# leodd/Lifted-Hybrid-Variational-Inference

Hardware: AMD Instinct MI355X
Metric: lbp_sweeps_per_sec_10M_edge_hybrid_mrf (higher is better)
Workload: dtype f64

## Files before the change

### include/lhvi.h

```cpp
#ifndef LHVI_H
#define LHVI_H

#include <stddef.h>
#include <stdint.h>

#ifdef __cplusplus
extern "C" {
#endif

#define LHVI_ABI_VERSION 31
#define LHVI_MAX_ARITY 6

#define LHVI_OK 0
#define LHVI_E_ARG (-1)
#define LHVI_E_LAUNCH (-2)
#define LHVI_E_UNSUPPORTED (-3)
#define LHVI_E_NODEVICE (-4)
#define LHVI_E_NOT_PD (-5)

#define LHVI_POT_GENERIC 0
#define LHVI_POT_TABLE 1
#define LHVI_POT_GAUSSIAN 2
#define LHVI_POT_QUADRATIC 3
#define LHVI_POT_HYBRID_QUADRATIC 4
#define LHVI_POT_LINEAR_GAUSSIAN 5
#define LHVI_POT_X2 6
#define LHVI_POT_XY 7
#define LHVI_POT_MLN 8
#define LHVI_POT_MLN_HARD 9
#define LHVI_POT_IMAGE_NODE 10
#define LHVI_POT_IMAGE_EDGE 11

typedef struct lhvi_graph {
    int32_t V, F, E, nnz;
    const int32_t* fac_ptr;
    const int32_t* edge_var;
    const int32_t* edge_fac;
    const int32_t* edge_canon;
    const int32_t* var_ptr;
    const int32_t* var_edge;
    const double* edge_count;
    const int32_t* fac_pot;
    const double* var_value;
    const int32_t* var_dom;
    const double* var_mult;
    const double* fac_mult;
    int32_t D;
    const int32_t* dom_cont;
    const double* dom_lo;
    const double* dom_hi;
    const int32_t* dom_ptr;
    const double* dom_val;
    const double* edge_value;
    const int32_t* slot_var;
    const int32_t* hub_vars;
    int32_t n_hubs;
} lhvi_graph_t;
#define LHVI_HUB_DEGREE 64

typedef struct lhvi_pots {
    int32_t P;
    const int32_t* kind;
    const int32_t* off;
    const double* param;
    int32_t interpreted;
} lhvi_pots_t;

int lhvi_version(void);
const char* lhvi_strerror(int code);
int lhvi_last_hip_error(void);
int lhvi_device_count(void);


int lhvi_gabp_init(const lhvi_graph_t* g, double* f2v, double* v2f, void* stream);
int lhvi_gabp_v2f(const lhvi_graph_t* g, const double* f2v, double* v2f, void* stream);
int lhvi_gabp_f2v(const lhvi_graph_t* g, const lhvi_pots_t* pots, const double* v2f, double* f2v, void* stream);
int lhvi_gabp_run(const lhvi_graph_t* g, const lhvi_pots_t* pots, double* f2v, double* v2f, int iterations, void* stream);
typedef struct lhvi_gabp_plan {
    const int32_t* pslot;
    const int32_t* info;
    const double* count;
    int32_t n_hub_rows;
    const int32_t* rec;
    const double* pot_words;
    const int32_t* seg;
    int32_t n_seg;
} lhvi_gabp_plan_t;
size_t lhvi_gabp_pull_workspace_bytes(const lhvi_graph_t* g);
int lhvi_gabp_pull(const lhvi_graph_t* g, const lhvi_pots_t* pots, const lhvi_gabp_plan_t* plan, const double* v_prev,
                   double* v_next, int first, void* stream);
int lhvi_gabp_run_pull(const lhvi_graph_t* g, const lhvi_pots_t* pots, const lhvi_gabp_plan_t* plan, double* f2v, double* v2f,
                       int iterations, void* ws, size_t ws_bytes, void* stream);

int lhvi_gabp_graph_create(const lhvi_graph_t* g, const lhvi_pots_t* pots, const lhvi_gabp_plan_t* plan, double* f2v, double* v2f,
                           double* mu_var, int iterations, void* ws, size_t ws_bytes, void** handle_out);
int lhvi_gabp_graph_launch(void* handle, void* stream);
int lhvi_gabp_graph_destroy(void* handle);

int lhvi_gabp_marginals(const lhvi_graph_t* g, const double* f2v, double* mu_var, void* stream);

size_t lhvi_log_likelihood_workspace_bytes(const lhvi_graph_t* g);
int lhvi_log_likelihood(const lhvi_graph_t* g, const lhvi_pots_t* pots, const double* x, double* out, void* ws, size_t ws_bytes,
                        void* stream);


#define LHVI_PBP_EP 1u
#define LHVI_PBP_EPBP_DISCRETE 2u
#define LHVI_PBP_SKIP_TERMS 16u
#define LHVI_PBP_LEAVE_ROOM 256u
#define LHVI_PBP_CQ 512u
#define LHVI_PBP_BOUNDARY_TOTALS 2048u
#define LHVI_PBP_NO_UNIQ 4096u
#define LHVI_PBP_V2F_RECORDS 8192u
#define LHVI_PBP_WIDE_PAIRS 16384u
#define LHVI_PBP_SHARE_CUS 32768u
#define LHVI_PBP_NO_GRID 128u
#define LHVI_PBP_FUSED_RECORDS16 131072u
#define LHVI_PBP_F2V_HEAVY 262144u
#define LHVI_PBP_F2V_SMALL 524288u
#define LHVI_PBP_F2V_PAIR 1048576u
#define LHVI_PBP_F2V_FAST 2097152u
#define LHVI_PBP_F2V_CQ 4194304u
#define LHVI_PBP_F2V_GENERIC 8388608u
#define LHVI_PBP_F2V_ALL (LHVI_PBP_F2V_HEAVY | LHVI_PBP_F2V_SMALL | LHVI_PBP_F2V_PAIR | LHVI_PBP_F2V_FAST | LHVI_PBP_F2V_CQ | LHVI_PBP_F2V_GENERIC)
#define LHVI_PBP_POW2_GROUPS 65536u

typedef struct lhvi_pbp {
    int32_t n;
    int32_t T;
    uint32_t flags;
    double var_threshold;
    double max_log_value;
    const double* particles;
    const double* old_particles;
    const int32_t* np;
    const uint8_t* uniq;
    const double* q;
    const int32_t* fast_edges;
    int32_t n_fast;
    const int32_t* generic_edges;
    int32_t n_generic;
    int32_t generic_pts_log2;
    const void* fast_desc;
    const void* heavy_desc;
    int32_t n_heavy;
    const void* light_desc;
    int32_t n_light;
    const int32_t* bslot;
    const int32_t* brow_ptr;
    const int64_t* brow_off;
    const int32_t* brow_peer;
    const double* recv;
    int32_t rank;
    const double* var_degree;
    int32_t var_lo, var_hi;
    uint32_t* f2v_ticket;
    const int32_t* prop_desc;
    int32_t n_prop_desc;
    const void* pair_desc;
    int32_t n_pair;
    const void* cq_desc;
    int32_t n_cq;
    const int32_t* v2f_wide;
    int32_t n_v2f_wide;
    const int32_t* v2f_narrow;
    int32_t n_v2f_narrow;
    const int32_t* v2f_hub;
    int32_t n_v2f_hub;
    const int32_t* v2f_mid16;
    int32_t n_v2f_mid16;
    const int32_t* v2f_mid32;
    int32_t n_v2f_mid32;
    const int32_t* prop_hub;
    int32_t n_prop_hub;
    double* prop_partial;
    const int32_t* resample_vars;
    int32_t n_resample_vars;
    const void* small16_desc;
    int32_t n_small16;
    const void* small32_desc;
    int32_t n_small32;
    const int64_t* halo_off;
    double* halo_buf;
} lhvi_pbp_t;

#define LHVI_PBP_DESC_BYTES 128
#define LHVI_PBP_TICKET_WORDS 16
#define LHVI_PBP_TICKET_COUNTERS 8
int lhvi_pbp_describe(const lhvi_graph_t* g, const lhvi_pots_t* pots, const lhvi_pbp_t* s, const int32_t* edges, int32_t count,
                      void* desc_out, void* stream);
int lhvi_pbp_describe_cq(const lhvi_graph_t* g, const lhvi_pots_t* pots, const lhvi_pbp_t* s, const int32_t* edges, int32_t count,
                         void* desc_out, void* stream);
int lhvi_pbp_var_sum(const lhvi_graph_t* g, const lhvi_pbp_t* s, const double* f2v, double* out, void* stream);
int lhvi_pbp_domain_grid(const lhvi_graph_t* g, const lhvi_pbp_t* s, double* x, void* stream);
int lhvi_pbp_refine_grid(const lhvi_graph_t* g, const lhvi_pbp_t* s, const double* logb, double* x, double* best, double* best_val,
                         void* stream);
int lhvi_debug_exp(const double* x, double* y, int64_t n, void* stream);
int lhvi_debug_exp_acc(const double* x, const double* c, double* y, int64_t n, void* stream);
int lhvi_debug_exp_acc_floor(const double* x, const double* c, double* y, int64_t n, void* stream);
// ... 409 lines not shown
```

### lifted-hybrid-variational-inference_amd/csrc/fastmath.hpp

```cpp
#pragma once
#include "common.hpp"

namespace lhvi {

#include "exp_table.inc"
constexpr int EXP_TAB_N = 1 << LHVI_EXP_TABLE_BITS;

__device__ __forceinline__ double exp_core(double t, const double* __restrict__ tab ) {
    const double MAGIC = LHVI_SCONST(6755399441055744.0);
    const double u = fma(t, LHVI_SCONST(LHVI_EXP_INV_STEP), MAGIC);
    const int nn = __double2loint(u);
    const double kd = u - MAGIC;
    double r = fma(kd, LHVI_SCONST(-LHVI_EXP_STEP_HI), t);
    r = fma(kd, LHVI_SCONST(-LHVI_EXP_STEP_LO), r);
    double p = fma(r, LHVI_SCONST(1.6666666666666666667e-1), 0.5);
    p = fma(p, r, 1.0);
    p = fma(p, r, 1.0);
    return ldexp(tab[nn & (EXP_TAB_N - 1)] * p, nn >> LHVI_EXP_TABLE_BITS);
}

__device__ __forceinline__ void load_exp_table(double* __restrict__ tab) {
    for (int i = threadIdx.x; i < EXP_TAB_N; i += blockDim.x) tab[i] = EXP_TAB[i];
    __syncthreads();
}

struct ExpShift { double magic, scale; };

__device__ __forceinline__ ExpShift exp_shift(double C) {
    const double MAGIC = 6755399441055744.0;
    ExpShift o;
    o.magic = fma(C, LHVI_EXP_INV_STEP, MAGIC);
    const double kd = o.magic - MAGIC;
    double r = fma(kd, -LHVI_EXP_STEP_HI, C);
    r = fma(kd, -LHVI_EXP_STEP_LO, r);
    double p = fma(r, 1.6666666666666666667e-1, 0.5);
    p = fma(p, r, 1.0);
    o.scale = fma(p, r, 1.0);
    return o;
}

__device__ __forceinline__ double exp_accumulate(double acc, double t, double magic, const double* __restrict__ tab) {
    double u;
    asm("v_fma_f64 %0, %1, %2, %3" : "=v"(u) : "v"(t), "s"((double)LHVI_EXP_INV_STEP), "v"(magic));
    const int nn = __double2loint(u);
    const double kd = u - magic;
    const double r = fma(kd, -LHVI_EXP_STEP_HI, t);
    double p = fma(r, 1.6666666666666666667e-1, 0.5);
    p = fma(p, r, 1.0);
    p = fma(p, r, 1.0);
    return fma(ldexp(tab[nn & (EXP_TAB_N - 1)], nn >> LHVI_EXP_TABLE_BITS), p, acc);
}

struct ExpShiftFloor { double magic, scale; };

__device__ __forceinline__ void round_down_on() { asm volatile("s_setreg_imm32_b32 hwreg(HW_REG_MODE, 2, 2), 2\n\ts_nop 1" ::: "memory"); }
__device__ __forceinline__ void round_down_off() { asm volatile("s_setreg_imm32_b32 hwreg(HW_REG_MODE, 2, 2), 0\n\ts_nop 1" ::: "memory"); }

__device__ __forceinline__ ExpShiftFloor exp_shift_floor(double C) {
    const double MAGIC = 6755399441055744.0;
    ExpShiftFloor o;
    const double m = fma(C, LHVI_EXP_INV_STEP, MAGIC);
    const double kd = m - MAGIC;
    double r = fma(kd, -LHVI_EXP_STEP_HI, C);
    r = fma(kd, -LHVI_EXP_STEP_LO, r);
    double p = fma(r, 1.6666666666666666667e-1, 0.5);
    p = fma(p, r, 1.0);
    o.scale = fma(p, r, 1.0) * LHVI_EXPF_SCALE;
    o.magic = 844424930131968.0 + (kd - (double)(24 << LHVI_EXP_TABLE_BITS));
    return o;
}

__device__ __forceinline__ double exp_accumulate_floor(double acc, double s, double magic, const double* __restrict__ tab) {
    double u;
    asm volatile("v_add_f64 %0, %1, %2" : "=v"(u) : "v"(s), "v"(magic));
    const int nn = __double2loint(u);
    const double f = __builtin_amdgcn_fract(s);
    double p = fma(f, LHVI_SCONST(LHVI_EXPF_RHO), 1.0);
    p = fma(p, f, LHVI_SCONST(LHVI_EXPF_K1));
    p = fma(p, f, LHVI_SCONST(LHVI_EXPF_K0));
    const double entry = *reinterpret_cast<const double*>(reinterpret_cast<const char*>(tab) + (nn & ((EXP_TAB_N - 1) << 3)));
    return fma(ldexp(entry, nn >> (LHVI_EXP_TABLE_BITS + 3)), p, acc);
}

constexpr int LOG_TAB_N = 1 << LHVI_LOG_TABLE_BITS;
struct LogRec { double inv_c, log_c; };

__device__ __forceinline__ void load_log_table(LogRec* __restrict__ tab) {
    for (int i = threadIdx.x; i < LOG_TAB_N; i += blockDim.x) { tab[i].inv_c = LOG_TAB[2 * i]; tab[i].log_c = LOG_TAB[2 * i + 1]; }
}

__device__ __forceinline__ double log_table(double x, const LogRec* __restrict__ tab) {
    const int e = __builtin_amdgcn_frexp_exp(x);
    const double m = __builtin_amdgcn_frexp_mant(x);
    const LogRec c = tab[(__double2hiint(m) >> (20 - LHVI_LOG_TABLE_BITS)) & (LOG_TAB_N - 1)];
    const double r = fma(m, c.inv_c, -1.0);
    double q = fma(r, LHVI_SCONST(1.0 / 7.0), LHVI_SCONST(-1.0 / 6.0));
    q = fma(q, r, LHVI_SCONST(1.0 / 5.0));
    q = fma(q, r, -0.25);
    q = fma(q, r, LHVI_SCONST(1.0 / 3.0));
    q = fma(q, r, -0.5);
    const double l = fma(r * r, q, r);
    const double y = fma((double)e, LHVI_SCONST(LHVI_LN2), c.log_c + l);
    return x == __builtin_huge_val() ? x : y;
}

}
```

### lifted-hybrid-variational-inference_amd/csrc/pbp.hip

```cpp
#include "common.hpp"
#include "potential.hpp"
#include "fastmath.hpp"
#include "cq.hpp"
#include "gk21.hpp"

namespace lhvi {

__device__ __forceinline__ double wave_sum(double v) { return dpp_wave_reduce(v, SumOp()); }
__device__ __forceinline__ double wave_max(double v) { return dpp_wave_reduce(v, MaxOp()); }
__device__ __forceinline__ int wave_sum_i(int v) {
#pragma unroll
    for (int off = 32; off > 0; off >>= 1) v += __shfl_xor(v, off);
    return v;
}

constexpr double PAD_LOG_TERM = -6.0e5;

__host__ __device__ __forceinline__ int var_first(const lhvi_pbp_t& s) { return s.var_hi > s.var_lo ? s.var_lo : 0; }
__host__ __device__ __forceinline__ int var_limit(const lhvi_graph_t& g, const lhvi_pbp_t& s) { return s.var_hi > s.var_lo ? s.var_hi : g.V; }

__device__ __forceinline__ double norm_pdf_std(double x, double mu, double sig) {
    const double u = (x - mu) / sig;
    return exp(-u * u * 0.5) / (2.506628274631 * sig);
}
// ... 507 lines not shown
            d.pad[0] = cont_target ? 1 : 2;
        }
    }
    return d;
}

__global__ void __launch_bounds__(BLOCK) pbp_describe_kernel(lhvi_graph_t g, lhvi_pots_t pots, lhvi_pbp_t s,
                                                            const int32_t* __restrict__ edges, int count,
                                                            FastDesc* __restrict__ out) {
    const int i = blockIdx.x * BLOCK + threadIdx.x;
    if (i < count) out[i] = make_fast_desc(g, pots, s, edges[i]);
}

#define LHVI_WAVE_SYNC() do { __builtin_amdgcn_fence(__ATOMIC_ACQ_REL, "wavefront"); __builtin_amdgcn_wave_barrier(); } while (0)

enum { MODE_CONST = 0, MODE_VARK = 1, MODE_DISC = 2 };
struct AB { double a, b; };

template <int MODE>
__device__ __forceinline__ double fast_term(double acc, const AB* __restrict__ sh, const double* __restrict__ shk,
                                            const double* __restrict__ tab, int j, double X1, double X2, double magic) {
    const AB r = sh[j];
    double t;
    if (MODE == MODE_VARK) t = fma(shk[j], X2, fma(r.b, X1, r.a));
    else t = fma(r.b, fma(r.b, X2, X1), r.a);
    return exp_accumulate(acc, t, magic, tab);
}

template <int MODE>
__device__ __forceinline__ double fast_accumulate_uniform(const AB* __restrict__ sh, const double* __restrict__ shk,
                                                          const double* __restrict__ tab, int jn_, double X1, double X2, double C) {
    const int jn = __builtin_amdgcn_readfirstlane(jn_);
    const ExpShift sft = exp_shift(C);
    double acc0 = 0.0, acc1 = 0.0;
    int j = 0;
    for (; j + 2 <= jn; j += 2) {
        acc0 = fast_term<MODE>(acc0, sh, shk, tab, j, X1, X2, sft.magic);
        acc1 = fast_term<MODE>(acc1, sh, shk, tab, j + 1, X1, X2, sft.magic);
    }
    if (j < jn) acc0 = fast_term<MODE>(acc0, sh, shk, tab, j, X1, X2, sft.magic);
    return (acc0 + acc1) * sft.scale;
}

#define LHVI_PIN1(a) do { if (PIN) asm volatile("" : "+v"(a)); } while (0)
#define LHVI_PIN2(a, b) do { if (PIN) asm volatile("" : "+v"(a), "+v"(b)); } while (0)
template <int UNROLL = 4, bool PIN = false>
__device__ __forceinline__ double fast_accumulate_floor(const AB* __restrict__ sh, const double* __restrict__ tab, int jn_, double X1,
                                                        double C) {
    const int jn = __builtin_amdgcn_readfirstlane(jn_);
    LHVI_PIN1(C);
    ExpShiftFloor sft = exp_shift_floor(C);
    LHVI_PIN2(sft.magic, sft.scale);
    double acc0 = 0.0, acc1 = 0.0;
    int j = 0;
    round_down_on();
    if (UNROLL == 4) {
        double acc2 = 0.0, acc3 = 0.0;
        for (; j + 4 <= jn; j += 4) {
            const AB r0 = sh[j], r1 = sh[j + 1], r2 = sh[j + 2], r3 = sh[j + 3];
            acc0 = exp_accumulate_floor(acc0, fma(r0.b, X1, r0.a), sft.magic, tab);
            acc1 = exp_accumulate_floor(acc1, fma(r1.b, X1, r1.a), sft.magic, tab);
            acc2 = exp_accumulate_floor(acc2, fma(r2.b, X1, r2.a), sft.magic, tab);
            acc3 = exp_accumulate_floor(acc3, fma(r3.b, X1, r3.a), sft.magic, tab);
        }
        if (j < jn) { const AB r0 = sh[j]; acc0 = exp_accumulate_floor(acc0, fma(r0.b, X1, r0.a), sft.magic, tab); }
        if (j + 1 < jn) { const AB r1 = sh[j + 1]; acc1 = exp_accumulate_floor(acc1, fma(r1.b, X1, r1.a), sft.magic, tab); }
        if (j + 2 < jn) { const AB r2 = sh[j + 2]; acc2 = exp_accumulate_floor(acc2, fma(r2.b, X1, r2.a), sft.magic, tab); }
        acc0 += acc2; acc1 += acc3;
        LHVI_PIN2(acc0, acc1);
        round_down_off();
        return (acc0 + acc1) * sft.scale;
    }
    for (; j + 2 <= jn; j += 2) {
        const AB r0 = sh[j], r1 = sh[j + 1];
        acc0 = exp_accumulate_floor(acc0, fma(r0.b, X1, r0.a), sft.magic, tab);
        acc1 = exp_accumulate_floor(acc1, fma(r1.b, X1, r1.a), sft.magic, tab);
    }
    if (j < jn) { const AB r0 = sh[j]; acc0 = exp_accumulate_floor(acc0, fma(r0.b, X1, r0.a), sft.magic, tab); }
    LHVI_PIN2(acc0, acc1);
    round_down_off();
    return (acc0 + acc1) * sft.scale;
}

__global__ void __launch_bounds__(BLOCK) pbp_f2v_fast_kernel(lhvi_graph_t g, lhvi_pots_t pots, lhvi_pbp_t s,
                                                            const double* __restrict__ v2f, double* __restrict__ f2v,
                                                            const FastDesc* __restrict__ descs,
                                                            const double* __restrict__ param) {
    __shared__ AB sh_all[BLOCK / WAVE][WAVE];
    __shared__ double shk_all[BLOCK / WAVE][WAVE];
    __shared__ double sh_tab[EXP_TAB_N];
    __shared__ LogRec sh_log[LOG_TAB_N];
    load_log_table(sh_log);
    load_exp_table(sh_tab);
    const int wid = __builtin_amdgcn_readfirstlane(threadIdx.x >> 6);
    const int lane = threadIdx.x & 63;
    AB* sh = sh_all[wid];
    double* shk = shk_all[wid];
    const int nitems = s.fast_edges ? s.n_fast : g.E;
    const int nwaves = gridDim.x * (BLOCK / WAVE);
    const int n = s.n, S = s.n + s.T;
    for (int item = blockIdx.x * (BLOCK / WAVE) + wid; item < nitems; item += nwaves) {
        FastDesc d;
        if (descs) d = descs[item];
        else d = make_fast_desc(g, pots, s, s.fast_edges ? s.fast_edges[item] : item);
        if (d.cls != EDGE_FAST_CONT && d.cls != EDGE_FAST_DISC) continue;
        const double* __restrict__ par = param + d.par_off;
        const int np = d.np, npts = d.np + d.T, nj = d.nj;
        const bool partner_hidden = is_hidden(d.pval);
        double* out = f2v + (int64_t)d.e * S;

        double y0 = d.pval, m0 = 0.0;
        if (partner_hidden && lane < nj) { y0 = s.old_particles[(int64_t)d.pv * n + lane]; m0 = v2f[(int64_t)d.pce * n + lane]; }
        double xr[2] = {0.0, 0.0};
#pragma unroll
        for (int r = 0; r < 2; ++r) {
            const int rem = npts - 64 * r;
            if (rem > 0) {
                int lw = 6;
                if (rem <= 32) { lw = 0; while ((1 << lw) < rem) ++lw; }
                const int pl = lane & ((1 << lw) - 1), pp = 64 * r + pl;
                if (pl < rem) xr[r] = pp < np ? s.particles[(int64_t)d.tv * n + pp] : g.dom_val[d.gb + pp - np];
            }
        }

        const int mode = d.cls == EDGE_FAST_DISC ? MODE_DISC : (d.kind == LHVI_POT_HYBRID_QUADRATIC ? MODE_VARK : MODE_CONST);
        double kconst = 0.0;
        if (mode == MODE_CONST) { Quad2 q; quad2_of(d.kind, par, 0, q); kconst = d.pos == 0 ? q.a00 : q.a11; }
        auto stage = [&](int j0, int jn, double y, double m) {
            LHVI_WAVE_SYNC();
            {
                AB r;
                r.a = PAD_LOG_TERM; r.b = 0.0;
                double kk = 0.0;
                if (lane < jn) {
                    if (d.cls == EDGE_FAST_CONT) {
                        Quad2 q;
                        quad2_of(d.kind, par, (d.kind == LHVI_POT_HYBRID_QUADRATIC) ? (int)y : 0, q);
                        if (d.pos == 0) { r.a = (q.a11 * y + q.b1) * y + q.c + m; r.b = q.axy * y + q.b0; kk = q.a00; }
                        else            { r.a = (q.a00 * y + q.b0) * y + q.c + m; r.b = q.axy * y + q.b1; kk = q.a11; }
                    } else { r.a = m; r.b = y; }
                }
                if (mode == MODE_CONST) { r.a *= LHVI_EXP_INV_STEP; r.b *= LHVI_EXP_INV_STEP; }
                sh[lane] = r;
                if (mode == MODE_VARK) shk[lane] = kk;
            }
            LHVI_WAVE_SYNC();
        };
        const bool single_tile = nj <= 64;
        if (single_tile) stage(0, nj, y0, m0);

        for (int p0 = 0; p0 < npts; p0 += 64) {
            const int rem = npts - p0;
            int lw = 6;
            if (rem <= 32) { lw = 0; while ((1 << lw) < rem) ++lw; }
            const int width = 1 << lw, split = 64 >> lw, sub = lane >> lw, pl = lane & (width - 1);
            const int p = p0 + pl;
            const bool valid = pl < rem;
            double xv = 0.0;
            if (p0 == 0) xv = xr[0];
            else if (p0 == 64) xv = xr[1];
            else if (valid) xv = p < np ? s.particles[(int64_t)d.tv * n + p] : g.dom_val[d.gb + p - np];
            double X1 = 0.0, X2 = 0.0, C = 0.0;
            if (valid) {
                if (d.cls == EDGE_FAST_CONT) { X1 = xv; X2 = xv * xv; C = kconst * X2; }
                else {
                    const int nst = (int)par[2];
// ... 332 lines not shown
                                                             double* __restrict__ f2v, const HeavyDesc* __restrict__ descs,
                                                             int nitems) {
    __shared__ AB sh_all[HEAVY_BLOCK / WAVE][WAVE];
    __shared__ double sh_tab[EXP_TAB_N];
    __shared__ LogRec sh_log[LOG_TAB_N];
    load_log_table(sh_log);
    load_exp_table(sh_tab);
    const int wid = __builtin_amdgcn_readfirstlane(threadIdx.x >> 6);
    const int lane = threadIdx.x & 63;
    AB* sh = sh_all[wid];
    const int n = s.n, S = s.n + s.T;
    WorkCursor<8, HEAVY_BLOCK / WAVE> cur;
    const auto ticket = [] { return heavy_arg_reload<uint32_t*>(offsetof(HeavyArgs, f2v_ticket)); };
    if (!cur.start(ticket, nitems, lane)) return;
    int n_grid = 0, n_direct = 0;
    struct { int32_t e, nj, np, T, gb, grid; double ay, by, c, axy, bx, kx, gx0, gh; } d;
    HeavyHead hn = descs[cur.item].h;
    HeavyData h = heavy_fetch(hn, s, v2f, lane);
    for (;;) {
        d.e = hn.e; d.nj = hn.nj; d.np = hn.np; d.T = hn.T; d.gb = hn.gb; d.grid = hn.grid;
        {
            const HeavyCoef k = descs[cur.item].k;
            d.ay = k.ay; d.by = k.by; d.c = k.c; d.axy = k.axy; d.bx = k.bx; d.kx = k.kx; d.gx0 = k.gx0; d.gh = k.gh;
        }
        const int nxt = cur.next();
        const bool more = nxt < cur.limit;
        hn = descs[__builtin_amdgcn_readfirstlane(min(nxt, cur.limit - 1))].h;
        const int np = d.np, nj = d.nj;
        const auto out = scalar_row(f2v + (int64_t)d.e * S);
        const double kconst = d.kx;
        const bool eligible = grid_eligible(d.grid, nj, d.T);
        bool grid_path = eligible && !(s.flags & (LHVI_PBP_SKIP_TERMS | LHVI_PBP_NO_GRID));
        AB mine;
        mine.a = PAD_LOG_TERM; mine.b = 0.0;
        LHVI_WAVE_SYNC();
        {
            if (lane < nj) {
                const double y = h.y;
                mine.a = (d.ay * y + d.by) * y + d.c + h.m;
                mine.b = d.axy * y + d.bx;
            }
            AB scaled;
            scaled.a = mine.a * LHVI_EXP_INV_STEP; scaled.b = mine.b * LHVI_EXP_INV_STEP;
            sh[lane] = scaled;
        }
        LHVI_WAVE_SYNC();
        if (grid_path) {
            const double X = fmax(fabs(d.gx0), fabs(fma((double)(d.T - 1), d.gh, d.gx0)));
            const double bound = fma(fabs(mine.b) + fabs(kconst) * X, X, fabs(mine.a));
            grid_path = __ballot(lane < nj && !(bound < GRID_MAX_EXPONENT)) == 0;
            if (grid_path) ++n_grid; else ++n_direct;
        }
        const int npts = eligible ? np : np + d.T;
        const double x0 = h.x0, x1 = h.x1;
        if (more) h = heavy_fetch(hn, s, v2f, lane);
        if (grid_path) {
            double gv = exp_core(fma(mine.b, d.gx0, mine.a), sh_tab);
            const double q = exp_core(mine.b * d.gh, sh_tab);
            double qr[4];
            grid_rows_ratios(q, qr);
            const double q2 = q * q, q4 = q2 * q2;
            for (int t0 = 0; t0 < d.T; t0 += 32) {
                const double sum = grid_sums32_rows(gv, qr, q4, t0 + 32 < d.T, lane);
                const int t = t0 + grid_rows_owned_point(lane);
                if (t < d.T && !(lane & 1)) {
                    const double xt = fma((double)t, d.gh, d.gx0);
                    row_store(out, (uint32_t)(n + t), sum > 0.0 ? fma(kconst * xt, xt, log_table(sum, sh_log)) : -700.0);
                }
            }
        } else if (eligible) {
#pragma nounroll
            for (int t0 = 0; t0 < d.T; t0 += 64) {
                const int rem = d.T - t0;
                const int lw = round_log2_width(rem);
                const int width = 1 << lw, split = 64 >> lw, sub = lane >> lw, pl = lane & (width - 1);
                const bool valid = pl < rem;
                const double X1 = valid ? heavy_arg_reload<const double*>(offsetof(HeavyArgs, dom_val))[d.gb + t0 + pl] : 0.0, C = kconst * X1 * X1;
                const int chunk = (s.flags & LHVI_PBP_SKIP_TERMS) ? 0 : (nj + split - 1) >> (6 - lw);
                double acc = fast_accumulate_floor<LHVI_HEAVY_UNROLL>(sh + sub * chunk, sh_tab, chunk, X1, C);
                for (int off = width; off < 64; off <<= 1) acc += __shfl_xor(acc, off);
                if (valid && sub == 0) row_store(out, (uint32_t)(n + t0 + pl), acc > 0.0 ? log_table(acc, sh_log) : -700.0);
            }
        }
#pragma nounroll
        for (int r = 0; r < 2; ++r) {
            const int rem = npts - 64 * r;
            if (rem <= 0) break;
            const int lw = round_log2_width(rem);
            const int width = 1 << lw, split = 64 >> lw, sub = lane >> lw, pl = lane & (width - 1);
            const int p = 64 * r + pl;
            const bool valid = pl < rem;
            const double xv = r == 0 ? x0 : x1;
            const double X1 = valid ? xv : 0.0, C = kconst * X1 * X1;
            const int chunk = (s.flags & LHVI_PBP_SKIP_TERMS) ? 0 : (nj + split - 1) >> (6 - lw);
            double acc = fast_accumulate_floor<LHVI_HEAVY_UNROLL>(sh + sub * chunk, sh_tab, chunk, X1, C);
            for (int off = width; off < 64; off <<= 1) acc += __shfl_xor(acc, off);
            if (valid && sub == 0) row_store(out, (uint32_t)(p < np ? p : n + (p - np)), acc > 0.0 ? log_table(acc, sh_log) : -700.0);
        }
        if (!more) break;
        cur.advance(nxt, lane, ticket);
    }
    uint32_t* stats = heavy_arg_reload<uint32_t*>(offsetof(HeavyArgs, stats));
    if (stats && lane == 0) { atomicAdd(stats, (uint32_t)n_grid); atomicAdd(stats + 1, (uint32_t)n_direct); }
}

#ifndef LHVI_SMALL_WAVES
#define LHVI_SMALL_WAVES 6
#endif
#ifndef LHVI_SMALL_WAVES10
#define LHVI_SMALL_WAVES10 5
#endif
#ifndef LHVI_SMALL_WAVES2
#define LHVI_SMALL_WAVES2 5
#endif
template <int W, int PPL = 1>
__global__ void __launch_bounds__(BLOCK) __attribute__((amdgpu_waves_per_eu(PPL == 2 ? LHVI_SMALL_WAVES2 : W == 10 ? LHVI_SMALL_WAVES10 : LHVI_SMALL_WAVES, 8))) pbp_f2v_small_kernel(lhvi_graph_t g, lhvi_pbp_t s, const double* __restrict__ v2f,
                                                            double* __restrict__ f2v, const FastDesc* __restrict__ descs, int nitems) {
    using Geo = SmallGeom<W>;
    constexpr int G = Geo::G;
    constexpr int GS = PPL * W + 1;
    constexpr int SH_AB = G * GS > Geo::BUF_AB ? G * GS : Geo::BUF_AB;
    __shared__ AB sh_all[BLOCK / WAVE][SH_AB];
    __shared__ double sh_tab[EXP_TAB_N];
    __shared__ LogRec sh_log[LOG_TAB_N];
    load_log_table(sh_log);
    load_exp_table(sh_tab);
    const int wid = __builtin_amdgcn_readfirstlane(threadIdx.x >> 6);
    const int lane = threadIdx.x & 63;
    const bool lane_ok = lane < G * W;
    const int grp = lane_ok ? lane / W : G - 1, gl = lane_ok ? lane % W : W - 1;
    AB* sh = sh_all[wid];
    const AB* mine_recs = sh + grp * GS;
    const int n = s.n, S = s.n + s.T;
    const int nsteps = (nitems + G - 1) / G;
    const int nwaves = gridDim.x * (BLOCK / WAVE);
    for (int step = blockIdx.x * (BLOCK / WAVE) + wid; step < nsteps; step += nwaves) {
        const int idx = step * G + grp;
        const bool live = idx < nitems && lane_ok;
        union { FastDesc d; int4 q[sizeof(FastDesc) / 16]; } u;
        {
            const int4* dp = reinterpret_cast<const int4*>(descs + min(idx, nitems - 1));
#pragma unroll
            for (int k = 0; k < (int)(sizeof(FastDesc) / 16); ++k) u.q[k] = dp[k];
        }
        const int touch = reinterpret_cast<const int*>(descs + min((step + nwaves) * G + grp, nitems - 1))[0];
        const FastDesc& d = u.d;
        const int e = d.e, tv = d.tv, nj = d.nj, np = d.np, T = d.T, gb = d.gb;
        const double pval = d.pval, kx = d.kx;
        const int npts = np + T;
        double yl[PPL], ml[PPL];
#pragma unroll
        for (int pp = 0; pp < PPL; ++pp) {
            const int jl = min(gl + pp * W, nj - 1);
            yl[pp] = s.old_particles[(int64_t)d.pv * n + jl]; ml[pp] = v2f[(int64_t)d.pce * n + jl];
        }
        double xs[3];
#pragma unroll
        for (int r = 0; r < 3; ++r) {
            const int p = r * W + gl;
            const double* src = p < np ? s.particles + ((int64_t)tv * n + p) : g.dom_val + (gb + max(min(p - np, T - 1), 0));
            xs[r] = *src;
        }
        const bool hidden_partner = is_hidden(pval);
        double ua[PPL], ub[PPL];
        AB rec[PPL];
#pragma unroll
        for (int pp = 0; pp < PPL; ++pp) {
            const double y = hidden_partner ? yl[pp] : pval, m = hidden_partner ? ml[pp] : 0.0;
            ua[pp] = PAD_LOG_TERM; ub[pp] = 0.0;
            if (gl + pp * W < nj) {
                ua[pp] = (d.ay * y + d.by) * y + d.c + m;
                ub[pp] = d.axy * y + d.bx;
            }
            rec[pp].a = ua[pp] * LHVI_EXP_INV_STEP; rec[pp].b = ub[pp] * LHVI_EXP_INV_STEP;
        }
        const double gx0 = d.pad2[0], gh = d.pad2[1];
        bool gok = false;
        if (d.pad[1] && T <= GRID_MAX_T && !(s.flags & (LHVI_PBP_SKIP_TERMS | LHVI_PBP_NO_GRID))) {
            const double X = fmax(fabs(gx0), fabs(fma((double)(T - 1), gh, gx0)));
            bool mine_bad = false;
// ... 2095 lines not shown
```

### lifted-hybrid-variational-inference_amd/lhvi/_abi.py

```python
from __future__ import annotations

import ctypes as C
import os

import numpy as np

_HERE = os.path.dirname(os.path.abspath(__file__))
LIB_PATH = os.environ.get('LHVI_LIB') or os.path.join(os.path.dirname(_HERE), 'csrc', 'liblhvi.so')

c_i32p = C.c_void_p
c_f64p = C.c_void_p


class LhviError(RuntimeError):
    pass


class GraphStruct(C.Structure):
    _fields_ = [
        ('V', C.c_int32), ('F', C.c_int32), ('E', C.c_int32), ('nnz', C.c_int32),
        ('fac_ptr', C.c_void_p), ('edge_var', C.c_void_p), ('edge_fac', C.c_void_p), ('edge_canon', C.c_void_p),
        ('var_ptr', C.c_void_p), ('var_edge', C.c_void_p), ('edge_count', C.c_void_p), ('fac_pot', C.c_void_p),
        ('var_value', C.c_void_p), ('var_dom', C.c_void_p), ('var_mult', C.c_void_p), ('fac_mult', C.c_void_p),
        ('D', C.c_int32),
        ('dom_cont', C.c_void_p), ('dom_lo', C.c_void_p), ('dom_hi', C.c_void_p), ('dom_ptr', C.c_void_p),
        ('dom_val', C.c_void_p), ('edge_value', C.c_void_p), ('slot_var', C.c_void_p),
        ('hub_vars', C.c_void_p), ('n_hubs', C.c_int32),
    ]


class GabpPlanStruct(C.Structure):
    _fields_ = [('pslot', C.c_void_p), ('info', C.c_void_p), ('count', C.c_void_p), ('n_hub_rows', C.c_int32), ('rec', C.c_void_p), ('pot_words', C.c_void_p), ('seg', C.c_void_p), ('n_seg', C.c_int32)]


class PotsStruct(C.Structure):
    _fields_ = [('P', C.c_int32), ('kind', C.c_void_p), ('off', C.c_void_p), ('param', C.c_void_p), ('interpreted', C.c_int32)]


class PbpStruct(C.Structure):
    _fields_ = [
        ('n', C.c_int32), ('T', C.c_int32), ('flags', C.c_uint32),
        ('var_threshold', C.c_double), ('max_log_value', C.c_double),
        ('particles', C.c_void_p), ('old_particles', C.c_void_p), ('np', C.c_void_p), ('uniq', C.c_void_p),
        ('q', C.c_void_p),
        ('fast_edges', C.c_void_p), ('n_fast', C.c_int32), ('generic_edges', C.c_void_p), ('n_generic', C.c_int32),
        ('generic_pts_log2', C.c_int32), ('fast_desc', C.c_void_p), ('heavy_desc', C.c_void_p), ('n_heavy', C.c_int32), ('light_desc', C.c_void_p), ('n_light', C.c_int32),
        ('bslot', C.c_void_p), ('brow_ptr', C.c_void_p), ('brow_off', C.c_void_p), ('brow_peer', C.c_void_p),
        ('recv', C.c_void_p), ('rank', C.c_int32), ('var_degree', C.c_void_p),
        ('var_lo', C.c_int32), ('var_hi', C.c_int32),
        ('f2v_ticket', C.c_void_p),
        ('prop_desc', C.c_void_p), ('n_prop_desc', C.c_int32),
        ('pair_desc', C.c_void_p), ('n_pair', C.c_int32),
        ('cq_desc', C.c_void_p), ('n_cq', C.c_int32),
        ('v2f_wide', C.c_void_p), ('n_v2f_wide', C.c_int32), ('v2f_narrow', C.c_void_p), ('n_v2f_narrow', C.c_int32),
        ('v2f_hub', C.c_void_p), ('n_v2f_hub', C.c_int32),
        ('v2f_mid16', C.c_void_p), ('n_v2f_mid16', C.c_int32), ('v2f_mid32', C.c_void_p), ('n_v2f_mid32', C.c_int32),
        ('prop_hub', C.c_void_p), ('n_prop_hub', C.c_int32), ('prop_partial', C.c_void_p),
        ('resample_vars', C.c_void_p), ('n_resample_vars', C.c_int32),
        ('small16_desc', C.c_void_p), ('n_small16', C.c_int32), ('small32_desc', C.c_void_p), ('n_small32', C.c_int32),
        ('halo_off', C.c_void_p), ('halo_buf', C.c_void_p),
    ]


class ViStruct(C.Structure):
    _fields_ = [
        ('K', C.c_int32), ('T', C.c_int32), ('Dmax', C.c_int32), ('quirks', C.c_int32),
        ('gh_x', C.c_void_p), ('gh_w', C.c_void_p), ('w', C.c_void_p), ('eta_c', C.c_void_p), ('eta_d', C.c_void_p),
        ('obs_var', C.c_void_p), ('var_N', C.c_void_p),
        ('fac_list', C.c_void_p), ('n_cc', C.c_int32), ('n_grp3', C.c_int32), ('n_grp6', C.c_int32), ('n_rest3', C.c_int32),
        ('n_rest6', C.c_int32), ('n_tiny', C.c_int32), ('tiny_par_words', C.c_int32), ('edge_axis', C.c_void_p),
    ]


class ViOptStruct(C.Structure):
    _fields_ = [(n, C.c_void_p) for n in ('w_tau', 'w', 'eta_c', 'tau_d', 'eta_d', 'm_w', 's_w', 'm_c', 's_c', 'm_d', 's_d',
                                          'g_w', 'g_c', 'g_d', 'fe')] + \
               [(n, C.c_double) for n in ('lr', 'b1', 'b2', 'eps', 'var_min')] + [('t', C.c_int32)]


PBP_EP = 1
PBP_EPBP_DISCRETE = 2
PBP_SKIP_TERMS = 16
PBP_NO_GRID = 128
PBP_LEAVE_ROOM = 256
PBP_BOUNDARY_TOTALS = 2048
PBP_CQ = 512
PBP_NO_UNIQ = 4096
PBP_V2F_RECORDS = 8192
PBP_WIDE_PAIRS = 16384
PBP_SHARE_CUS = 32768
PBP_POW2_GROUPS = 65536
PBP_FUSED_RECORDS16 = 131072
PBP_F2V_HEAVY = 262144
PBP_F2V_SMALL = 524288
PBP_F2V_PAIR = 1048576
PBP_F2V_FAST = 2097152
PBP_F2V_CQ = 4194304
PBP_F2V_GENERIC = 8388608
PBP_F2V_ALL = PBP_F2V_HEAVY | PBP_F2V_SMALL | PBP_F2V_PAIR | PBP_F2V_FAST | PBP_F2V_CQ | PBP_F2V_GENERIC
ABI_VERSION = 31
PBP_DESC_BYTES = 128
COLOR_HASH, COLOR_SORT = 0, 1
HUB_DEGREE = 64
VI_GROUP_SLOTS, VI_GROUP_COMP, VI_TINY_NODES, VI_TINY_K, VI_TINY_PAR = 24, 48, 32, 2, 3072

class MwsStruct(C.Structure):
    _fields_ = [('T', C.c_int32), ('max_flips', C.c_int32), ('epsilon', C.c_double), ('noise_std', C.c_double),
                ('seed', C.c_uint64), ('try_id', C.c_void_p), ('disc', C.c_void_p), ('n_disc', C.c_int32),
                ('num', C.c_void_p), ('n_num', C.c_int32), ('fac_class', C.c_void_p), ('x', C.c_void_p), ('best_x', C.c_void_p),
                ('cur_score', C.c_void_p), ('best_score', C.c_void_p), ('status', C.c_void_p), ('err_flip', C.c_void_p),
                ('rec_score', C.c_void_p), ('rec_zero', C.c_void_p), ('rec_ticks', C.c_void_p)] + \
               [(n, C.c_void_p) for n in ('rp_init', 'rp_clause', 'rp_walk', 'rp_walk_k', 'rp_noise', 'rp_post', 'out_score',
                                          'out_unsat', 'out_winner', 'out_accept', 'out_val')]


class ExactStruct(C.Structure):
    _fields_ = [('Nd', C.c_int32), ('Nc', C.c_int32), ('M', C.c_int64), ('dstates', C.c_void_p), ('dstride', C.c_void_p),
                ('n_quad', C.c_int32), ('quad_ptr', C.c_void_p), ('quad_desc', C.c_void_p), ('quad_par', C.c_void_p),
                ('n_tab', C.c_int32), ('tab_ptr', C.c_void_p), ('tab_desc', C.c_void_p), ('tab_par', C.c_void_p)]


class GibbsStruct(C.Structure):
    _fields_ = [('ex', ExactStruct), ('dstate_off', C.c_void_p), ('vt_ptr', C.c_void_p), ('vt_fac', C.c_void_p),
                ('vh_ptr', C.c_void_p), ('vh_fac', C.c_void_p), ('n_hyb', C.c_int32), ('hyb_quad', C.c_void_p),
                ('hyb_off', C.c_void_p), ('table_doubles', C.c_int32), ('max_states', C.c_int32), ('table_scratch', C.c_void_p),
                ('disc_block_its', C.c_int32), ('num_burnin', C.c_int32), ('num_samples', C.c_int32), ('seed', C.c_uint64)]


class FgibbsStruct(C.Structure):
    _fields_ = [('n_colours', C.c_int32), ('col_ptr', C.c_void_p), ('col_var', C.c_void_p), ('hub_ptr', C.c_void_p),
                ('hub_var', C.c_void_p), ('max_shrink', C.c_int32), ('hub_degree', C.c_int32), ('num_burnin', C.c_int32),
                ('num_samples', C.c_int32), ('thin', C.c_int32), ('seed', C.c_uint64), ('u', C.c_void_p), ('init_x', C.c_void_p),
                ('cnt_off', C.c_void_p), ('counts', C.c_void_p), ('sum1', C.c_void_p), ('sum2', C.c_void_p),
                ('keep_row', C.c_void_p), ('samples', C.c_void_p), ('stuck', C.c_void_p), ('capped', C.c_void_p),
                ('evals', C.c_void_p)]


FGIBBS_MAX_STATES = 16
E_NOT_PD = -5
EXACT_MAX_NC = 64
GAUSS_EXACT_NB = 64
GAUSS_CHAIN_MAX_BLOCK = 128

MIX_MAX_K, MIX_TILE, MIX_ROWS = 128, 64, 4
MIX_GAUSSIAN, MIX_VI = 0, 1
GMFIT_MAX_K = 16
GMKL_MAX_PANELS = 1024
GMKL_LOGQ = C.CFUNCTYPE(C.c_double, C.c_double, C.c_int64, C.c_void_p)
VI_GAUSSIAN_PDF = 2
NPVI_MAX_K, NPVI_MAX_SLOTS = 16, 24


class NpviOptStruct(C.Structure):
    _fields_ = [(n, C.c_void_p) for n in ('tau', 'theta_c', 'rho', 'm_tau', 's_tau', 'm_c', 's_c', 'm_rho', 's_rho', 'g_tau', 'g_c',
                                          'g_rho', 'obj', 'w', 'eta_c', 'eta_d', 'mu_lo', 'mu_hi')] + \
               [('lvar_lo', C.c_double), ('lvar_hi', C.c_double), ('var_count', C.c_void_p), ('fac_count', C.c_void_p)] + \
               [(n, C.c_double) for n in ('lr', 'b1', 'b2', 'eps')] + [('t', C.c_int32), ('max_slots', C.c_int32), ('max_arity', C.c_int32)]


class MixStruct(C.Structure):
    _fields_ = [('V', C.c_int32), ('K', C.c_int32), ('Dmax', C.c_int32), ('nstates', C.c_void_p), ('logw', C.c_void_p),
                ('rec', C.c_void_p), ('lpi', C.c_void_p), ('pi', C.c_void_p)]


LBFGSB_FUN = C.CFUNCTYPE(C.c_double, C.POINTER(C.c_double), C.c_void_p)

_G, _P, _S, _VI = C.POINTER(GraphStruct), C.POINTER(PotsStruct), C.POINTER(PbpStruct), C.POINTER(ViStruct)
_GP = C.POINTER(GabpPlanStruct)
_MX = C.POINTER(MixStruct)
_NO = C.POINTER(NpviOptStruct)
_vp, _i32, _i64, _u32, _u64, _f64, _sz = C.c_void_p, C.c_int32, C.c_int64, C.c_uint32, C.c_uint64, C.c_double, C.c_size_t

SIGNATURES = {
    'lhvi_version': (C.c_int, []),
    'lhvi_strerror': (C.c_char_p, [C.c_int]),
    'lhvi_last_hip_error': (C.c_int, []),
    'lhvi_device_count': (C.c_int, []),
    'lhvi_gabp_init': (C.c_int, [_G, _vp, _vp, _vp]),
    'lhvi_gabp_v2f': (C.c_int, [_G, _vp, _vp, _vp]),
    'lhvi_gabp_f2v': (C.c_int, [_G, _P, _vp, _vp, _vp]),
    'lhvi_gabp_run': (C.c_int, [_G, _P, _vp, _vp, C.c_int, _vp]),
    'lhvi_gabp_marginals': (C.c_int, [_G, _vp, _vp, _vp]),
    'lhvi_gabp_pull_workspace_bytes': (C.c_size_t, [_G]),
# ... 319 lines not shown
```

### lifted-hybrid-variational-inference_amd/lhvi/pbp.py

```python
from __future__ import annotations

import os
from math import e, log, sqrt

import numpy as np

from . import _abi, pbp_plan, pbp_query
from .flat import flatten

_F2V_LONG = _abi.PBP_F2V_HEAVY | _abi.PBP_F2V_SMALL
_F2V_SHORT = _abi.PBP_F2V_PAIR | _abi.PBP_F2V_FAST | _abi.PBP_F2V_CQ | _abi.PBP_F2V_GENERIC
F2V_SCHEDULES = {
    'one': (('main', _abi.PBP_F2V_ALL, 0, False),),
    'timed': (('main', _F2V_LONG, 0, True), ('main', _F2V_SHORT, 0, False)),
    'overlap': (('side', _F2V_SHORT, 0, False), ('main', _F2V_LONG, _abi.PBP_SHARE_CUS, True)),
}


def _stream(st):
    return _abi.stream_ptr() if st is None else st


class _ParticleSweep:
    var_threshold = 3
    max_log_value = 700
    _epbp_discrete = True
    verbose = False
    listed_proposal = True
    dynamic_f2v = True
    paired_light = True
    cq_routing = True
    small_f2v = True
    long_grid_min_edges = 1 << 16
    listed_resample = True
    sliced_proposal = True
    prop_slice = 64
    packed_v2f = True
    overlap_f2v = True
    overlap_min_heavy = 1 << 16
    fused_var_kernel = True
    fused_max_particles = 64
    exact_queries = False
    map_mode = 'fminbound'
    var_gid = None
    _side = None
    _query_f2v = None
    _stable_partition = False
    _ground = None

    def _setup(self, graph_like, flat=None, edge_key=None, sides='vf', edge_skip=None, owned=None):
        flat = flat if flat is not None else flatten(graph_like, require_device_potentials=True)
        self.flat = flat
        self.dg = dg = _abi.DeviceGraph(flat)
        torch = _abi.require_gpu()
        n = self.n
        plan = pbp_plan.var_side_plan(flat, n, owned=owned, opts=self._plan_options())
        self.np_host, self.T = plan.np_host, plan.T
        S = n + self.T
        self.f2v = dg.zeros(flat.E, S)
        self.v2f = dg.zeros(flat.E, n)
        self.eta = dg.zeros(flat.E, 2)
        self.q_dev = dg.zeros(flat.V, 2)
        self.particles = dg.zeros(flat.V, n)
        self.old_particles = dg.zeros(flat.V, n)
        self.uniq = torch.zeros(flat.V, n, dtype=torch.uint8, device=dg.device)
        self.f2v_ticket = torch.zeros(16, dtype=torch.int32, device=dg.device)
        self.flags = (_abi.PBP_EP if self.proposal_approximation == 'EP' else 0) | \
                     (_abi.PBP_EPBP_DISCRETE if self._epbp_discrete else 0) | \
                     (_abi.PBP_CQ if self.cq_routing and bool((flat.pot_kind == 8).any()) else 0) | \
                     (_abi.PBP_POW2_GROUPS if os.environ.get('LHVI_PBP_POW2_GROUPS', '0') == '1' else 0) | \
                     plan.flags
        self._views, self._batched = {}, {}
        self._draws = 0
        self._static_rows = False
        self.var_lists = plan.on(_abi.upload(plan.host), dg.zeros(plan.n_prop_partial, 2) if plan.n_prop_partial else None)
        for name, value in self.var_lists.named().items():
            setattr(self, name, value)
        self._has_f_side = 'f' in sides
        self.f2v_lists = pbp_plan.F2vLists.empty(torch.zeros(1, dtype=torch.int32, device=dg.device))
        if self._has_f_side:
            cls = torch.zeros(max(flat.E, 1), dtype=torch.uint8, device=dg.device)
            _abi.check(_abi.lib().lhvi_pbp_classify(dg.g, dg.p, self._struct(), _abi.ptr(cls), _abi.stream_ptr()))
            self.f2v_lists = pbp_plan.f_side_plan(
                cls[:flat.E], flat, self.np_host, describe=self._describe,
                describe_cq=lambda edges: self._describe(edges, 'lhvi_pbp_describe_cq', 2 * _abi.PBP_DESC_BYTES),
                skip=None if edge_skip is None else _abi.to_dev(np.ascontiguousarray(edge_skip, dtype=bool)),
                key=None if edge_key is None else _abi.to_dev(np.ascontiguousarray(edge_key, dtype=np.int32)),
                paired_light=self.paired_light, small_f2v=self.small_f2v, long_grid_min_edges=self.long_grid_min_edges)
        for name, value in self.f2v_lists.named().items():
            setattr(self, name, value)

    def _describe(self, edges, entry='lhvi_pbp_describe', nbytes=_abi.PBP_DESC_BYTES):
        torch = _abi.require_gpu()
        k = int(edges.numel())
        desc = torch.empty(k * nbytes, dtype=torch.uint8, device=edges.device)
        _abi.check(getattr(_abi.lib(), entry)(self.dg.g, self.dg.p, self._struct(), _abi.ptr(edges), k, _abi.ptr(desc), _abi.stream_ptr()))
        return desc

    def _plan_options(self):
        env = os.environ.get
        return pbp_plan.PlanOptions(
            sampler_on_device=self.sampler == 'device', listed_proposal=self.listed_proposal, listed_resample=self.listed_resample,
            sliced_proposal=self.sliced_proposal, prop_slice=self.prop_slice, packed_v2f=self.packed_v2f,
            v2f_records=env('LHVI_PBP_V2F_REC', '1') != '0',
            fused=self.fused_var_kernel and env('LHVI_PBP_FUSED', '1') != '0',
            fused_max_particles=int(env('LHVI_PBP_FUSED_MAX', self.fused_max_particles)),
            fused_records16=env('LHVI_PBP_FUSED_REC16', '1') != '0')

    def _struct(self, var_range=None, leave_room=False):
        s = _abi.PbpStruct()
        s.n, s.T, s.flags = self.n, self.T, self.flags | (_abi.PBP_LEAVE_ROOM if leave_room else 0)
        s.var_threshold, s.max_log_value = float(self.var_threshold), float(self.max_log_value)
        s.particles, s.old_particles = _abi.ptr(self.particles), _abi.ptr(self.old_particles)
        s.uniq, s.q = _abi.ptr(self.uniq), _abi.ptr(self.q_dev)
        self.f2v_lists.install(s)
        if var_range is None:
            self.var_lists.install(s, self.listed_proposal)
        else:
            self.var_lists.install_range(s, *var_range)
        s.f2v_ticket = _abi.ptr(self.f2v_ticket) if self.dynamic_f2v else None
        return s

    def _launch_init(self, s, st=None):
        _abi.check(_abi.lib().lhvi_pbp_init(self.dg.g, s, _abi.ptr(self.eta), _abi.ptr(self.q_dev), _abi.ptr(self.f2v), _abi.ptr(self.v2f),
                                            _stream(st)))

    def _launch_v2f(self, s, st=None):
        _abi.check(_abi.lib().lhvi_pbp_v2f(self.dg.g, s, _abi.ptr(self.f2v), _abi.ptr(self.v2f), _stream(st)))

    def _launch_proposal(self, s, st=None):
        _abi.check(_abi.lib().lhvi_pbp_proposal(self.dg.g, s, _abi.ptr(self.f2v), _abi.ptr(self.eta), _abi.ptr(self.q_dev), _stream(st)))

    def _launch_proposal_partial(self, s, ph, st=None):
        _abi.check(_abi.lib().lhvi_pbp_proposal_partial(self.dg.g, s, _abi.ptr(self.f2v), _abi.ptr(self.eta), _abi.ptr(ph), _stream(st)))

    def _launch_proposal_finish(self, s, ph, st=None):
        _abi.check(_abi.lib().lhvi_pbp_proposal_finish(self.dg.g, s, _abi.ptr(ph), _abi.ptr(self.q_dev), _stream(st)))

    def _launch_draw(self, s, st=None):
        _abi.check(_abi.lib().lhvi_pbp_resample_uniq(self.dg.g, s, _abi.ptr(self.var_gid), int(self.seed), int(self._draws - 1),
                                                     _abi.ptr(self.particles), _abi.ptr(self.uniq), _stream(st)))

    def _launch_fused(self, s, st=None):
        l, F, st = _abi.lib(), self.var_lists.fused, _stream(st)
        args = (self.dg.g, s, _abi.ptr(self.f2v), _abi.ptr(self.v2f), _abi.ptr(self.eta), _abi.ptr(self.q_dev), _abi.ptr(self.var_gid),
                int(self.seed), int(self._draws), _abi.ptr(self.old_particles), _abi.ptr(self.uniq))
        if sum(F.counts):
            _abi.check(l.lhvi_pbp_var_fused(*args, _abi.ptr(F.desc), *F.counts, st))
        if F.desc64 is not None:
            _abi.check(l.lhvi_pbp_var_fused64(*args, _abi.ptr(F.desc64), *F.counts64, st))

    def _new_sample(self):
        self.old_particles, self.particles = self.particles, self.old_particles
# ... 918 lines not shown
```

Before: 71.40.

## Add split-wave heavy f2v accumulation for 64-particle rows using permlane32 swaps

For the heavy f2v kernel with exactly 64 particles and 64 points, the two 32-lane halves of each wave now each take half the term records for two particle values, swapped in with permlane32_swap. The halves are then combined with another swap. This replaces the two-round loop with width-based shuffle reductions, so there are fewer passes and fewer cross-lane reductions per row. It adds an env/flag escape hatch and a new ABI version, and it ties correctness to the 64/64 shape and to the row layout of the shared records.

```diff
diff --git a/include/lhvi.h b/include/lhvi.h
--- a/include/lhvi.h
+++ b/include/lhvi.h
@@ -8,7 +8,7 @@
 extern "C" {
 #endif
 
-#define LHVI_ABI_VERSION 31
+#define LHVI_ABI_VERSION 32
 #define LHVI_MAX_ARITY 6
 
 #define LHVI_OK 0
@@ -115,6 +115,7 @@
 #define LHVI_PBP_WIDE_PAIRS 16384u
 #define LHVI_PBP_SHARE_CUS 32768u
 #define LHVI_PBP_NO_GRID 128u
+#define LHVI_PBP_NO_SPLIT_ROUND 16777216u
 #define LHVI_PBP_FUSED_RECORDS16 131072u
 #define LHVI_PBP_F2V_HEAVY 262144u
 #define LHVI_PBP_F2V_SMALL 524288u
diff --git a/lifted-hybrid-variational-inference_amd/csrc/fastmath.hpp b/lifted-hybrid-variational-inference_amd/csrc/fastmath.hpp
--- a/lifted-hybrid-variational-inference_amd/csrc/fastmath.hpp
+++ b/lifted-hybrid-variational-inference_amd/csrc/fastmath.hpp
@@ -70,6 +70,20 @@
     return o;
 }
 
+__device__ __forceinline__ double exp_shift_floor_steps(double C) {
+    const double MAGIC = 6755399441055744.0;
+    const double m = fma(C, LHVI_EXP_INV_STEP, MAGIC);
+    return m - MAGIC;
+}
+__device__ __forceinline__ double exp_shift_floor_magic(double kd) { return 844424930131968.0 + (kd - (double)(24 << LHVI_EXP_TABLE_BITS)); }
+__device__ __forceinline__ double exp_shift_floor_rest(double C, double kd) {
+    double r = fma(kd, -LHVI_EXP_STEP_HI, C);
+    r = fma(kd, -LHVI_EXP_STEP_LO, r);
+    double p = fma(r, 1.6666666666666666667e-1, 0.5);
+    p = fma(p, r, 1.0);
+    return fma(p, r, 1.0);
+}
+
 __device__ __forceinline__ double exp_accumulate_floor(double acc, double s, double magic, const double* __restrict__ tab) {
     double u;
     asm volatile("v_add_f64 %0, %1, %2" : "=v"(u) : "v"(s), "v"(magic));
diff --git a/lifted-hybrid-variational-inference_amd/csrc/pbp.hip b/lifted-hybrid-variational-inference_amd/csrc/pbp.hip
--- a/lifted-hybrid-variational-inference_amd/csrc/pbp.hip
+++ b/lifted-hybrid-variational-inference_amd/csrc/pbp.hip
@@ -613,6 +613,51 @@
     return (acc0 + acc1) * sft.scale;
 }
 
+__device__ __forceinline__ double fast_accumulate_floor_split(const AB* __restrict__ sh, const double* __restrict__ tab, int nj_, double X,
+                                                              double kconst, int lane) {
+    const int iters = __builtin_amdgcn_readfirstlane((nj_ + 3) >> 2);
+    asm volatile("" : "+v"(lane));
+    const bool upper = lane >= 32;
+    double c_own = kconst * X * X;
+    asm volatile("" : "+v"(c_own));
+    double k_own = exp_shift_floor_steps(c_own);
+    const double m_own = exp_shift_floor_magic(k_own);
+    double xa, xb, ma, mb;
+    {
+        auto x_lo = __builtin_amdgcn_permlane32_swap(__double2loint(X), __double2loint(X), false, false);
+        auto x_hi = __builtin_amdgcn_permlane32_swap(__double2hiint(X), __double2hiint(X), false, false);
+        auto m_lo = __builtin_amdgcn_permlane32_swap(__double2loint(m_own), __double2loint(m_own), false, false);
+        auto m_hi = __builtin_amdgcn_permlane32_swap(__double2hiint(m_own), __double2hiint(m_own), false, false);
+        xa = __hiloint2double(x_hi[0], x_lo[0]); xb = __hiloint2double(x_hi[1], x_lo[1]);
+        ma = __hiloint2double(m_hi[0], m_lo[0]); mb = __hiloint2double(m_hi[1], m_lo[1]);
+    }
+    asm volatile("" : "+v"(ma), "+v"(mb), "+v"(c_own), "+v"(k_own));
+    const AB* __restrict__ mine = sh + (upper ? 1 : 0);
+    double a0 = 0.0, a1 = 0.0, b0 = 0.0, b1 = 0.0;
+    round_down_on();
+    asm volatile("" : "+v"(c_own), "+v"(k_own));
+    double scale = exp_shift_floor_rest(c_own, k_own);
+    asm volatile("" : "+v"(scale));
+    const auto step = [&](int m) {
+        const AB r0 = mine[4 * m], r1 = mine[4 * m + 2];
+        a0 = exp_accumulate_floor(a0, fma(r0.b, xa, r0.a), ma, tab);
+        b0 = exp_accumulate_floor(b0, fma(r0.b, xb, r0.a), mb, tab);
+        a1 = exp_accumulate_floor(a1, fma(r1.b, xa, r1.a), ma, tab);
+        b1 = exp_accumulate_floor(b1, fma(r1.b, xb, r1.a), mb, tab);
+    };
+    int m = 0;
+    for (; m + 2 <= iters; m += 2) { step(m); step(m + 1); }
+    if (m < iters) step(m);
+    a0 += a1; b0 += b1;
+    asm volatile("" : "+v"(a0), "+v"(b0));
+    round_down_off();
+    asm volatile("" : "+v"(a0), "+v"(b0), "+v"(scale));
+    scale *= LHVI_EXPF_SCALE;
+    auto lo = __builtin_amdgcn_permlane32_swap(__double2loint(a0), __double2loint(b0), false, false);
+    auto hi = __builtin_amdgcn_permlane32_swap(__double2hiint(a0), __double2hiint(b0), false, false);
+    return (__hiloint2double(hi[0], lo[0]) + __hiloint2double(hi[1], lo[1])) * scale;
+}
+
 __global__ void __launch_bounds__(BLOCK) pbp_f2v_fast_kernel(lhvi_graph_t g, lhvi_pots_t pots, lhvi_pbp_t s,
                                                             const double* __restrict__ v2f, double* __restrict__ f2v,
                                                             const FastDesc* __restrict__ descs,
@@ -1111,6 +1156,11 @@
                 if (valid && sub == 0) row_store(out, (uint32_t)(n + t0 + pl), acc > 0.0 ? log_table(acc, sh_log) : -700.0);
             }
         }
+        const uint32_t split_flags = heavy_arg_reload<uint32_t>(offsetof(HeavyArgs, flags));
+        if (np == 64 && npts == 64 && !(split_flags & (LHVI_PBP_SKIP_TERMS | LHVI_PBP_NO_SPLIT_ROUND))) {
+            const double acc = fast_accumulate_floor_split(sh, sh_tab, nj, x0, kconst, lane);
+            row_store(out, (uint32_t)lane, acc > 0.0 ? log_table(acc, sh_log) : -700.0);
+        } else {
 #pragma nounroll
         for (int r = 0; r < 2; ++r) {
             const int rem = npts - 64 * r;
@@ -1125,6 +1175,7 @@
             double acc = fast_accumulate_floor<LHVI_HEAVY_UNROLL>(sh + sub * chunk, sh_tab, chunk, X1, C);
             for (int off = width; off < 64; off <<= 1) acc += __shfl_xor(acc, off);
             if (valid && sub == 0) row_store(out, (uint32_t)(p < np ? p : n + (p - np)), acc > 0.0 ? log_table(acc, sh_log) : -700.0);
+        }
         }
         if (!more) break;
         cur.advance(nxt, lane, ticket);
diff --git a/lifted-hybrid-variational-inference_amd/lhvi/_abi.py b/lifted-hybrid-variational-inference_amd/lhvi/_abi.py
--- a/lifted-hybrid-variational-inference_amd/lhvi/_abi.py
+++ b/lifted-hybrid-variational-inference_amd/lhvi/_abi.py
@@ -91,6 +91,7 @@
 PBP_SHARE_CUS = 32768
 PBP_POW2_GROUPS = 65536
 PBP_FUSED_RECORDS16 = 131072
+PBP_NO_SPLIT_ROUND = 16777216
 PBP_F2V_HEAVY = 262144
 PBP_F2V_SMALL = 524288
 PBP_F2V_PAIR = 1048576
@@ -98,7 +99,7 @@
 PBP_F2V_CQ = 4194304
 PBP_F2V_GENERIC = 8388608
 PBP_F2V_ALL = PBP_F2V_HEAVY | PBP_F2V_SMALL | PBP_F2V_PAIR | PBP_F2V_FAST | PBP_F2V_CQ | PBP_F2V_GENERIC
-ABI_VERSION = 31
+ABI_VERSION = 32
 PBP_DESC_BYTES = 128
 COLOR_HASH, COLOR_SORT = 0, 1
 HUB_DEGREE = 64
diff --git a/lifted-hybrid-variational-inference_amd/lhvi/pbp.py b/lifted-hybrid-variational-inference_amd/lhvi/pbp.py
--- a/lifted-hybrid-variational-inference_amd/lhvi/pbp.py
+++ b/lifted-hybrid-variational-inference_amd/lhvi/pbp.py
@@ -69,6 +69,7 @@
                      (_abi.PBP_EPBP_DISCRETE if self._epbp_discrete else 0) | \
                      (_abi.PBP_CQ if self.cq_routing and bool((flat.pot_kind == 8).any()) else 0) | \
                      (_abi.PBP_POW2_GROUPS if os.environ.get('LHVI_PBP_POW2_GROUPS', '0') == '1' else 0) | \
+                     (_abi.PBP_NO_SPLIT_ROUND if os.environ.get('LHVI_PBP_SPLIT_ROUND', '1') == '0' else 0) | \
                      plan.flags
         self._views, self._batched = {}, {}
         self._draws = 0
```

Measured after the change: 72.60, median of 6. 1.7% higher.
